# mizeller/OnePose_ST

Hardware: AMD Instinct MI355X
Metric: query frames/sec (2D-3D match+PnP) @ 7k x 4800 d256; 1/2/4/8 GPU (higher is better)
Workload: dtype bf16x3 (split-bf16 MFMA, f32 accumulate)

## Files before the change

onepose_st_amd/csrc/frame.hip:

```cpp
#include "tile.h"
#include "onepose_hip.h"
#include "x3w8_internal.h"
#include <mutex>
#include <unordered_map>
#include <vector>

namespace {

constexpr int kSlots = 16;
struct FineJob {
    bool pending = false;
    hipStream_t s_main = nullptr, s_fine = nullptr, s_copy = nullptr;
    const float* ff = nullptr; long long fs_b = 0, fs_c = 0, fs_y = 0, fs_x = 0; int hf = 0, wf = 0;
    const float* desc_f = nullptr; long long desc_f_bs = 0, desc_f_cs = 0;
    const long long *b_ids = nullptr, *i_ids = nullptr, *j_ids = nullptr; const int* count = nullptr; int cap = 0;
    const float* mkc = nullptr; const void* w_fine = nullptr; int n_fine = 0; unsigned fine_cross_bits = 0; int fine_encoder_enable = 0;
    int wc = 0, stride = 0; float fine_scale = 0.f;
    float *expec = nullptr, *mk2d = nullptr;
    const float* qscale = nullptr;
    void* host_dst = nullptr; const void* result_src = nullptr; size_t host_bytes = 0;
};
struct Slot {
    hipEvent_t prep_done = nullptr, coarse_done = nullptr, fine_done = nullptr, ready = nullptr, enc_done = nullptr;
    int dev = -1;
    int gen = 0;
    bool recorded = false;
    FineJob job;
};
struct DevState {
    Slot slots[kSlots];
    int next = 0;
    std::unordered_map<hipStream_t, hipEvent_t> last_fine;
    std::unordered_map<hipStream_t, int> deferred;
};
std::mutex g_mu;
std::mutex g_launch_mu;
std::unordered_map<int, DevState> g_dev;

size_t up256(size_t v) { return (v + 255) & ~(size_t)255; }

int make_events(Slot& s, int dev) {
    if (s.ready && s.dev == dev) return 0;
    hipEvent_t* ev[5] = {&s.prep_done, &s.coarse_done, &s.fine_done, &s.ready, &s.enc_done};
    for (auto e : ev) {
        hipError_t rc = hipEventCreateWithFlags(e, e == &s.ready ? (hipEventDisableTiming | hipEventBlockingSync) : hipEventDisableTiming);
        if (rc != hipSuccess) return ophip_fail(rc, "hipEventCreateWithFlags(frame)");
    }
    s.dev = dev;
    return 0;
}

}

#define FR_CHECK(call)                                  \
    do {                                                \
        const int rc__ = (call);                        \
        if (rc__ != 0) return rc__;                     \
    } while (0)
#define FR_HIP(call, what)                              \
    do {                                                \
        const hipError_t e__ = (call);                  \
        if (e__ != hipSuccess) return ophip_fail(e__, what); \
    } while (0)

namespace {
int launch_fine_job(int dev, Slot& s, hipEvent_t after = nullptr) {
    FineJob& j = s.job;
    const hipStream_t on = j.s_fine;
    FR_HIP(hipStreamWaitEvent(on, after ? after : s.coarse_done, 0), "hipStreamWaitEvent(fine job)");
    if (j.qscale)
        FR_CHECK(ophip_fine_refine_bf16_scaled(j.ff, j.fs_b, j.fs_c, j.fs_y, j.fs_x, j.hf, j.wf, j.desc_f, j.desc_f_bs, j.desc_f_cs, j.b_ids, j.i_ids, j.j_ids,
                                               j.count, j.cap, j.mkc, j.w_fine, j.n_fine, j.fine_cross_bits, j.fine_encoder_enable, 3, j.wc, j.stride,
                                               j.fine_scale, j.expec, j.mk2d, nullptr, nullptr, j.qscale, on));
    else
    FR_CHECK(ophip_fine_refine_bf16(j.ff, j.fs_b, j.fs_c, j.fs_y, j.fs_x, j.hf, j.wf, j.desc_f, j.desc_f_bs, j.desc_f_cs, j.b_ids, j.i_ids, j.j_ids,
                                    j.count, j.cap, j.mkc, j.w_fine, j.n_fine, j.fine_cross_bits, j.fine_encoder_enable, 3, j.wc, j.stride,
                                    j.fine_scale, j.expec, j.mk2d, nullptr, nullptr, on));
    FR_HIP(hipEventRecord(s.fine_done, on), "hipEventRecord(fine)");
    FR_HIP(hipStreamWaitEvent(j.s_copy, s.fine_done, 0), "hipStreamWaitEvent(fine)");
    FR_HIP(hipMemcpyAsync(j.host_dst, j.result_src, j.host_bytes, hipMemcpyDeviceToHost, j.s_copy), "hipMemcpyAsync(result block)");
// ... 72 lines not shown
    L->feat2d_out = (d->n_coarse % 2 == 0) ? L->x2d : L->y2d;
    return 0;
}

namespace {
int frame_enqueue_impl(const ophip_frame_desc* d, const ophip_frame_layout_t* L, void* blob_,
                       const float* feat_c, const float* feat_f, long long fs_b, long long fs_c, long long fs_y, long long fs_x,
                       const float* kpts, long long kpts_bs, const float* desc_c, long long desc_c_bs,
                       const float* desc_f, long long desc_f_bs, long long desc_f_cs, const ophip_object_cache* obj, bool ext_main_only,
                       const unsigned char* qmask, const float* qscale,
                       void* host_dst, size_t host_bytes, void* s_main_, void* s_prep_, void* s_fine_, void* s_copy_,
                       int* slot_out) {
    if (!d || !L || !blob_ || !feat_c || !feat_f || !kpts || !desc_c || !desc_f || !host_dst || !s_fine_ || !s_copy_ || !slot_out)
        return ophip_bad_arg(__func__, "null pointer");
    if (host_bytes < 16 || host_bytes > L->result_bytes) return ophip_bad_arg(__func__, "host_bytes");
    const bool deep = obj && obj->y3d0;
    const float* x3d_external = (obj && !deep) ? obj->x3d : nullptr;
    const long long x3d_ext_bs = obj ? obj->x3d_bs : -1;
    if (obj && !deep && !obj->x3d) return ophip_bad_arg(__func__, "object cache without buffers");
    if (deep && (!obj->kv1 || (reinterpret_cast<uintptr_t>(obj->kv1) & 15))) return ophip_bad_arg(__func__, "object cache: kv1 missing or not 16-byte aligned");
    if (deep && (d->n_coarse < 2 || (d->coarse_cross_bits & 1u))) return ophip_bad_arg(__func__, "a cached first layer needs n_coarse >= 2 and a first layer of kind \"self\"");
    if ((L->x3d == 0) != (obj != nullptr)) return ophip_bad_arg(__func__, "x3d_external / object cache does not match the layout");
    {
        const size_t want = deep ? ((d->n_coarse % 2 == 0) ? L->y3d : L->z3d) : ((d->n_coarse % 2 == 0) ? (obj ? L->z3d : L->x3d) : L->y3d);
        if (L->feat3d_out != want) return ophip_bad_arg(__func__, "layout was made for another external_x3d mode");
    }
    char* blob = static_cast<char*>(blob_);
    hipStream_t s_main = (hipStream_t)s_main_, s_prep = (hipStream_t)s_prep_, s_fine = (hipStream_t)s_fine_, s_copy = (hipStream_t)s_copy_;
    const int B = d->B, N = d->N, M = d->M, cap = B * N;
    int dev = 0;
    FR_HIP(hipGetDevice(&dev), "hipGetDevice");
    const bool defer = defer_fine_enabled() && s_fine != s_main;
    std::lock_guard<std::mutex> launch_lock(g_launch_mu);
    Slot* slot;
    Slot* kept = nullptr;
// ... 8 lines not shown
        slot = &st.slots[idx];
        FR_CHECK(make_events(*slot, dev));
        stale_job = slot->job.pending;
    }
    if (stale_job) FR_CHECK(launch_fine_job(dev, *slot));
    {
        std::lock_guard<std::mutex> lk(g_mu);
        DevState& st = g_dev[dev];
        if (slot->recorded) prev_ready = slot->ready;
        auto it = st.last_fine.find(s_main);
        if (it != st.last_fine.end()) prev_fine = it->second;
        auto dt = st.deferred.find(s_main);
        if (dt != st.deferred.end()) kept = &st.slots[dt->second];
    }
    if (prev_ready) FR_HIP(hipEventSynchronize(prev_ready), "hipEventSynchronize(slot reuse)");
    {
        std::lock_guard<std::mutex> lk(g_mu);
        slot->recorded = false;
        gen = ++slot->gen;
    }
    struct AbandonGuard {
        Slot* slot; hipStream_t st[4]; bool armed = true;
        ~AbandonGuard() {
            if (!armed) return;
            for (hipStream_t s : st) if (s) (void)hipStreamSynchronize(s);
            std::lock_guard<std::mutex> lk(g_mu);
            slot->recorded = false;
            slot->job.pending = false;
        }
    } abandon{slot, {s_main, s_prep, s_fine, s_copy}};
    auto F = [&](size_t off) { return reinterpret_cast<float*>(blob + off); };
    auto I64 = [&](size_t off) { return reinterpret_cast<long long*>(blob + off); };

    hipStream_t sin = s_prep ? s_prep : s_main;
    OphipRange frame_range("ophip_frame_enqueue");
    struct StageRange {
        bool open = false;
        void next(const char* name) { if (open) ophip_range_pop(); ophip_range_push(name); open = true; }
        ~StageRange() { if (open) ophip_range_pop(); }
    } stage;
    stage.next("a1-a3 input kernels");
    static const bool prep_after_sim = [] { const char* e = getenv("OPHIP_FRAME_PREP_AFTER_SIM"); return e && e[0] == '1'; }();
    if (prep_after_sim && s_prep && kept) FR_HIP(hipStreamWaitEvent(s_prep, kept->enc_done, 0), "hipStreamWaitEvent(previous similarity)");
    float* x2d = F(L->x2d);
    FR_CHECK(ophip_pe_add_transpose(feat_c, d->pe, x2d, B, 256, M, sin));
    const float* ff = feat_f;
    if (L->ffcl) {
        FR_CHECK(ophip_transpose_cl(feat_f, F(L->ffcl), B, d->cf, d->hf * d->wf, sin));
        ff = F(L->ffcl);
        fs_b = (long long)d->hf * d->wf * d->cf; fs_c = 1; fs_y = (long long)d->wf * d->cf; fs_x = d->cf;
    }
    if (obj && obj->ready) {
        FR_HIP(hipStreamWaitEvent(s_main, (hipEvent_t)obj->ready, 0), "hipStreamWaitEvent(object cache)");
        if (s_prep) FR_HIP(hipStreamWaitEvent(s_prep, (hipEvent_t)obj->ready, 0), "hipStreamWaitEvent(object cache, input stream)");
    }
    float* x3d = x3d_external ? const_cast<float*>(x3d_external) : (deep ? nullptr : F(L->x3d));
    if (!obj) {
        if (d->w_kpt) FR_CHECK(ophip_kpt_encode(kpts, kpts_bs, desc_c, desc_c_bs, d->w_kpt, F(L->stats), x3d, B, N, sin));
// ... 158 lines not shown
extern "C" int ophip_frame_enqueue(const ophip_frame_desc* d, const ophip_frame_layout_t* L, void* blob,
                                   const float* feat_c, const float* feat_f, long long fs_b, long long fs_c, long long fs_y, long long fs_x,
                                   const float* kpts, long long kpts_bs, const float* desc_c, long long desc_c_bs,
                                   const float* desc_f, long long desc_f_bs, long long desc_f_cs, const float* x3d_external,
                                   void* host_dst, size_t host_bytes, void* s_main, void* s_prep, void* s_fine, void* s_copy, int* slot_out) {
    return ophip_frame_enqueue_padded(d, L, blob, feat_c, feat_f, fs_b, fs_c, fs_y, fs_x, kpts, kpts_bs, desc_c, desc_c_bs, desc_f, desc_f_bs, desc_f_cs,
                                      x3d_external, nullptr, nullptr, host_dst, host_bytes, s_main, s_prep, s_fine, s_copy, slot_out);
}

extern "C" int ophip_frame_enqueue_object(const ophip_frame_desc* d, const ophip_frame_layout_t* L, void* blob,
                                          const float* feat_c, const float* feat_f, long long fs_b, long long fs_c, long long fs_y, long long fs_x,
                                          const float* kpts, long long kpts_bs, const float* desc_c, long long desc_c_bs,
                                          const float* desc_f, long long desc_f_bs, long long desc_f_cs, const ophip_object_cache* object,
                                          const unsigned char* qmask, const float* qscale,
                                          void* host_dst, size_t host_bytes, void* s_main, void* s_prep, void* s_fine, void* s_copy, int* slot_out) {
    if (object && !object->x3d && !object->y3d0) return ophip_bad_arg(__func__, "object cache without buffers");
    return frame_enqueue_impl(d, L, blob, feat_c, feat_f, fs_b, fs_c, fs_y, fs_x, kpts, kpts_bs, desc_c, desc_c_bs, desc_f, desc_f_bs, desc_f_cs,
                              object, false, qmask, qscale, host_dst, host_bytes, s_main, s_prep, s_fine, s_copy, slot_out);
}

extern "C" int ophip_frame_wait(int ticket) {
    if (ticket < kSlots) return ophip_bad_arg(__func__, "not a ticket of ophip_frame_enqueue");
    const int slot = ticket % kSlots, gen = ticket / kSlots;
    int dev = 0;
    FR_HIP(hipGetDevice(&dev), "hipGetDevice");
    hipEvent_t ev;
    {
        std::lock_guard<std::mutex> launch_lock(g_launch_mu);
        Slot* kept = nullptr;
        {
            std::lock_guard<std::mutex> lk(g_mu);
            Slot& s = g_dev[dev].slots[slot];
            if (s.gen > gen) return 0;
            if (s.gen == gen && s.job.pending) kept = &s;
        }
        if (kept) FR_CHECK(launch_fine_job(dev, *kept));
    }
    {
        std::lock_guard<std::mutex> lk(g_mu);
        const Slot& s = g_dev[dev].slots[slot];
        if (s.gen > gen) return 0;
        if (s.gen < gen || !s.recorded) return ophip_bad_arg(__func__, "ticket of a frame that was never (completely) enqueued on this device");
        ev = s.ready;
    }
    FR_HIP(hipEventSynchronize(ev), "hipEventSynchronize(frame)");
    return 0;
}

extern "C" int ophip_frame_order_after_fine(void* compute_stream) {
    int dev = 0;
    FR_HIP(hipGetDevice(&dev), "hipGetDevice");
    hipEvent_t ev = nullptr;
    std::lock_guard<std::mutex> launch_lock(g_launch_mu);
    Slot* kept = nullptr;
    {
        std::lock_guard<std::mutex> lk(g_mu);
        DevState& st = g_dev[dev];
        auto dt = st.deferred.find((hipStream_t)compute_stream);
        if (dt != st.deferred.end()) kept = &st.slots[dt->second];
    }
// ... 11 lines not shown
```

onepose_st_amd/csrc/prep.hip:

```cpp
#include "tile.h"
#include "crop_pixel.h"

namespace {

__global__ __launch_bounds__(256) void pe_add_transpose_kernel(const float* __restrict__ feat, const float* __restrict__ pe,
                                                               float* __restrict__ out, int Cc, int M) {
    __shared__ float tile[32][33];
    const int tx = threadIdx.x & 31, ty = threadIdx.x >> 5;
    const int m0 = blockIdx.x * 32, c0 = blockIdx.y * 32, b = blockIdx.z;
    const float* f = feat + (size_t)b * Cc * M;
#pragma unroll
    for (int k = 0; k < 4; ++k) {
        const int c = c0 + ty + 8 * k, m = m0 + tx;
        tile[ty + 8 * k][tx] = (c < Cc && m < M) ? f[(size_t)c * M + m] : 0.f;
    }
    __syncthreads();
    float* o = out + (size_t)b * M * Cc;
#pragma unroll
    for (int k = 0; k < 4; ++k) {
        const int m = m0 + ty + 8 * k, c = c0 + tx;
        if (m < M && c < Cc) o[(size_t)m * Cc + c] = tile[tx][ty + 8 * k] + (pe ? pe[(size_t)m * Cc + c] : 0.f);
    }
}

// ... 172 lines not shown
        for (int m = 0; m < 4; ++m) {
            const int q = q0 + 8 * m;
            f32x4 v = {tile[4 * q][p], tile[4 * q + 1][p], tile[4 * q + 2][p], tile[4 * q + 3][p]};
            *reinterpret_cast<f32x4*>(dst + (size_t)(l0 + p) * 128 + 4 * q) = v;
        }
    }
}

__global__ __launch_bounds__(256) void crop_resize_kernel(const unsigned char* __restrict__ img, int H, int W, int x0, int y0, int wb, int hb,
                                                          int S, float* __restrict__ out) {
    const int X = blockIdx.x * 32 + (threadIdx.x & 31), Y = blockIdx.y * 8 + (threadIdx.x >> 5);
    if (X >= S || Y >= S) return;
    out[(size_t)Y * S + X] = crop_pixel(img, H, W, x0, y0, wb, hb, S, X, Y);
}

}

extern "C" int ophip_crop_resize_gray(const unsigned char* image, int H, int W, int x0, int y0, int x1, int y1, int S, float* out, void* stream) {
    if (!image || !out) return ophip_bad_arg(__func__, "null pointer");
    if (H < 1 || W < 1 || S < 1 || x1 <= x0 || y1 <= y0) return ophip_bad_arg(__func__, "bad sizes (need x1 > x0, y1 > y0)");
    OPHIP_LAUNCH("crop_resize", (hipStream_t)stream, crop_resize_kernel, dim3((S + 31) / 32, (S + 7) / 8), dim3(256), 0, (hipStream_t)stream,
                 image, H, W, x0, y0, x1 - x0, y1 - y0, S, out);
    OPHIP_CHECK_LAUNCH();
    return 0;
}

extern "C" int ophip_pe_add_transpose(const float* feat_nchw, const float* pe_nlc, float* out_nlc, int B, int C, int M, void* stream) {
    if (!feat_nchw || !out_nlc) return ophip_bad_arg(__func__, "null pointer");
    if (B < 1 || C < 1 || M < 1) return ophip_bad_arg(__func__, "bad sizes");
    OPHIP_LAUNCH("pe_add_transpose", (hipStream_t)stream, pe_add_transpose_kernel, dim3((M + 31) / 32, (C + 31) / 32, B), dim3(256), 0, (hipStream_t)stream,
// ... 40 lines not shown
```

onepose_st_amd/csrc/x3w8_internal.h:

```cpp
#pragma once

int ophip_x3w8_object_first(const float* x2d, float* y2d, int B, int L3d, int L2d, const void* wpack, const void* wpack_next, int kv_mode,
                            void* workspace, const unsigned char* mask2d, bool only_kv, void* stream);
int ophip_x3w8_object_second(const float* y3d0, long long y3d0_bs, const float* x2d, float* y3d, float* y2d, int B, int L3d, int L2d,
                             const void* wpack, const void* wpack_next, int is_cross, const void* kv1, long long kv1_bs,
                             void* workspace, void* frag3d, void* frag2d, const unsigned char* mask2d, void* stream);
int ophip_x3w8_layer_bs(const float* x3d, long long x3d_bs, const float* x2d, float* y3d, float* y2d, int B, int L3d, int L2d,
                        const void* wpack, const void* wpack_next, int is_cross, int kv_mode, int slot,
                        void* workspace, void* frag3d, void* frag2d, const unsigned char* mask2d, bool only_kv, void* stream);

bool ophip_coarse_two_pass(int B, int N, int M);

int ophip_coarse_sim_store(const float* feat0, const float* feat1, int B, int N, int M, float* conf, float* workspace,
                           const float** rowstat, float** rowbest, unsigned** colmax_bits, void* stream,
                           const unsigned char* mask0 = nullptr, const unsigned char* mask1 = nullptr);
int ophip_coarse_select_2d(const float* conf, int nspan, const float* points0, long long points_bstride, int B, int N, int M, int wi, int wc,
                           float thr, int border_rm, float scale, float* workspace, long long* b_ids, long long* i_ids, long long* j_ids,
                           float* mconf, float* mkpts0, float* mkpts1_c, long long* m_bids, unsigned char* gt_mask, int* count, void* stream,
                           const unsigned char* mask0 = nullptr, const unsigned char* mask1 = nullptr);
```

onepose_st_amd/model.py:

```python
from __future__ import annotations

import contextlib
import ctypes
import os
import weakref
from collections import namedtuple

import torch
import torch.nn as nn

from . import hip, host_math, ops, packing
from .backbone import build_backbone
from .backbone_hip import HipBackbone, pack_backbone
from .config import encoder_layer_names, validate_config
from .hip import bstride
from .lazy_conf import LazyConfMatrixBase
from .params import EncoderParams, load_matcher_checkpoint
from .rows import rows_encoder_layer


class _KeypointEncoderParams(nn.Module):

    def __init__(self, inp_dim, feature_dim, layers):
        super().__init__()
# ... 11 lines not shown


def _current_stream(dev):
    idx = dev.index
    if idx is None:
        return torch.cuda.current_stream(dev)
    raw = torch._C._cuda_getCurrentRawStream(idx)
    st = _stream_objs.get((idx, raw))
    if st is None:
        st = torch.cuda.current_stream(dev)
        if len(_stream_objs) >= 64:
            _stream_objs.clear()
        _stream_objs[(idx, raw)] = st
    return st


_NSPLIT = {"f32": 0, "bf16": 1, "bf16x3": 3}


def _side_stream(table, key, dev, priority=0, with_event=False):
    ent = table.get(key)
    if ent is None:
        if len(table) >= 16:
            table.pop(next(iter(table)))
        st = torch.cuda.Stream(device=dev, priority=priority)
        ent = table[key] = [st, None] if with_event else st
    return ent


def _dense(t):
# ... 54 lines not shown
        fp = config.get("hip_fine_precision")
        if fp is not None:
            if str(fp) not in ("bf16x3", "bf16"):
                raise ValueError(f"hip_fine_precision {fp!r}: expected 'bf16x3' or 'bf16'")
            os.environ["OPHIP_FINE_PRECISION"] = str(fp)
        self.hip_backbone = bool(config.get("hip_backbone", True)) and self.precision != "f32"
        self.lazy_reruns = 0
        self._packed = None
        self._packed_bb = None
        self.overlap_fine = bool(config.get("hip_overlap_fine", True))
        self._fine_streams = {}
        self._prep_streams = {}
        self._pe_cache = {}
        self.cache_object = bool(config.get("hip_cache_object", False))
        self._obj_cache = None
        self.conf_matrix_mode = str(config.get("hip_conf_matrix", "eager"))
        if self.conf_matrix_mode not in ("eager", "lazy"):
            raise ValueError(f"hip_conf_matrix {self.conf_matrix_mode!r}: expected 'eager' or 'lazy'")
        if self.conf_matrix_mode == "lazy" and self.precision == "f32":
            raise ValueError("hip_conf_matrix = 'lazy' needs a bf16 arithmetic mode (the exact-f32 mode always materialises conf_matrix)")
        self.frame_call = bool(config.get("hip_frame_call", os.environ.get("OPHIP_FRAME_CALL", "1") != "0"))
        self._frame_plans = {}
        self._plan_ids = set()
        weakref.finalize(self, ops.drop_frame_plans, self._plan_ids)
        self._frame_call_pending = set()

        pretrained = config["loftr_backbone"]["pretrained"]
        if pretrained is not None:
            ckpt = torch.load(pretrained, map_location="cpu", weights_only=True)["state_dict"]
            sub = {k[k.find("backbone") + len("backbone") + 1:]: v for k, v in ckpt.items() if "backbone" in k}
# ... 55 lines not shown

        def coarse(pack):
            return [pack(sd, f"loftr_coarse.layers.{i}.").to(device) for i in range(len(self.loftr_coarse.layer_names))]
        blocks = {"coarse": coarse(packing.pack_coarse_layer),
                  "fine": torch.cat([packing.pack_fine_layer(sd, f"loftr_fine.layers.{i}.") for i in range(n_fine)]).to(device)}
        if self.kpt_3d_pos_encoding is not None:
            blocks["kpt"] = packing.pack_keypoint_encoder(sd).to(device)
        if self.precision == "bf16":
            blocks["coarse_bf16"] = coarse(packing.pack_coarse_layer_bf16)
        if self.precision == "bf16x3":
            blocks["coarse_x3"] = coarse(packing.pack_coarse_layer_x3w8)
        if self.fine_full:
            blocks["fine_full"] = [{n: t.to(device) for n, t in packing.pack_fine_layer_full_x3(sd, f"loftr_fine.layers.{i}.").items()} for i in range(n_fine)]
        if self.precision != "f32":
            blocks["fine_bf16"] = packing.pack_fine_layers_bf16(sd, "loftr_fine.layers.", n_fine).to(device)
        self._packed = (key, blocks)
        return blocks

    def _backbone_blocks(self, device):
        tensors = list(self.backbone.state_dict().values())
        key = (str(device),) + tuple((t.data_ptr(), t._version) for t in tensors)
        if self._packed_bb is None or self._packed_bb[0] != key:
            self._packed_bb = (key, pack_backbone(self.backbone.state_dict(), device))
        return self._packed_bb[1]

    def _pe_table(self, h, w, device):
        k = (h, w, str(device))
        if k not in self._pe_cache:
            self._pe_cache[k] = host_math.pe_table(self.config["loftr_coarse"]["d_model"], h, w, self._pe_shape).to(device)
        return self._pe_cache[k]
# ... 20 lines not shown
        if not self.hip_backbone:
            raise RuntimeError("hip_backbone is disabled for this model (exact-f32 mode or config['hip_backbone'] = False)")
        if not img.is_cuda:
            raise hip.HipLibraryError("OnePosePlus_model runs on the HIP device only (no CPU fallback): move the "
                                      "model and its inputs to 'cuda'")
        B, _, H, W = img.shape
        pe = self._pe_table(H // 8, W // 8, img.device) if self._pe_enable else None
        fc, ff = HipBackbone(self.precision).forward(self._backbone_blocks(img.device), img, pe)
        return (fc.view(B, H // 8, W // 8, fc.shape[2]).permute(0, 3, 1, 2), ff.view(B, H // 2, W // 2, ff.shape[2]).permute(0, 3, 1, 2))

    def forward_features(self, data, feat_c, feat_f, image_hw=None, want_fine_debug=False):
        self.enqueue_features(data, feat_c, feat_f, image_hw, want_fine_debug).finish()

    @torch.no_grad()
    def enqueue_features(self, data, feat_c, feat_f, image_hw=None, want_fine_debug=False, host_copy=False, _pe_applied=False,
                         inputs_ready=False, _force_eager=False):
        fi = self._frame_inputs(data, feat_c, feat_f, image_hw)
        main = _current_stream(fi.dev)
        fkey = (str(fi.dev), main.cuda_stream)
        lazy = self.conf_matrix_mode == "lazy" and not _force_eager
        rerun = (lambda: self.enqueue_features(data, feat_c, feat_f, image_hw, want_fine_debug, host_copy, _pe_applied, False, True)) if lazy else None
        if (self.frame_call and self.precision == "bf16x3" and not self.coarse_full and not self.fine_full and self.overlap_fine and not _pe_applied and not want_fine_debug
                and not self.debug and bool(self.config["fine_matching"]["enable"])
                and (self.kpt_3d_pos_encoding is not None or fi.B == 1 or fi.desc_in_d.shape[0] == fi.B)
                and len(self.loftr_coarse.layer_names) <= 16):
            return self._enqueue_frame_call(data, feat_c, feat_f, fi, main, fkey, host_copy, inputs_ready, lazy, rerun)
        if fkey in self._frame_call_pending:
            self._frame_call_pending.discard(fkey)
            hip.call("ophip_frame_order_after_fine", ctypes.c_void_p(main.cuda_stream))
        x2d, x3d, ff, ff_strides = self._input_stage(fi, feat_c, feat_f, main, fkey, _pe_applied, inputs_ready)
        x3d, x2d = self._coarse_encoder_stage(fi, x3d, x2d, main, fkey)
        if self.debug:
            data["_feat3d_c"], data["_feat2d_c"] = x3d, x2d
        cb, select = self._coarse_matching_stage(data, fi, x3d, x2d, main, lazy)
        pend = self._fine_stage(data, fi, cb, select, ff, ff_strides, main, fkey, want_fine_debug, host_copy)
        pend._rerun = rerun
        return pend

    def _frame_inputs(self, data, feat_c, feat_f, image_hw):
        if not feat_c.is_cuda:
            raise hip.HipLibraryError("OnePosePlus_model runs on the HIP device only (no CPU fallback): move the "
# ... 301 lines not shown
            d.w_kpt = W["kpt"].data_ptr() if self.kpt_3d_pos_encoding is not None else None
            for li in range(len(names_c)):
                d.w_coarse[li] = W["coarse_x3"][li].data_ptr()
            d.w_fine = W["fine_bf16"].data_ptr()
            L = hip.FrameLayout()
            hip.call("ophip_frame_layout", ctypes.byref(d), 1 if transpose_fine else 0, ext_mode, ctypes.byref(L))
            if len(self._frame_plans) >= 8:
                old_id = self._frame_plans.pop(next(iter(self._frame_plans)))[2]
                self._plan_ids.discard(old_id)
                ops.drop_frame_plan(old_id)
            pid = ops.register_frame_plan(d, L, keep_alive=(W, pe))
            self._plan_ids.add(pid)
            plan = self._frame_plans[pkey] = (d, L, pid, (W, pe))
        return plan

    def _enqueue_frame_call(self, data, feat_c, feat_f, fi, main, fkey, host_copy, inputs_ready, lazy=False, rerun=None):
        B, N, M, dev, kpts_d, desc_in_d, desc_fine_d, qmask, qscale = fi.B, fi.N, fi.M, fi.dev, fi.kpts_d, fi.desc_in_d, fi.desc_fine_d, fi.qmask, fi.qscale
        x3d_ext = None
        if self.cache_object or (B > 1 and kpts_d.shape[0] == 1 and desc_in_d.shape[0] == 1):
            x3d_ext = self._object_cache_entry(fi, main, masked=qmask is not None, keep=self.cache_object)
        fc = _dense(feat_c)
        ff = feat_f if feat_f.dtype == torch.float32 else feat_f.float()
        transpose_fine = ff.stride(1) != 1
        if transpose_fine:
            ff = ff.contiguous()
        ext_mode = 0 if x3d_ext is None else (2 if x3d_ext["y3d0"] is not None else 1)
        d, L, plan_id = self._frame_plan(fi, ff.shape[1], transpose_fine, ext_mode, data["q_hw_i"][0], lazy)[:3]

        fine_entry = self._fine_streams.get(fkey)
        if fine_entry is None:
            fine_entry = _side_stream(self._fine_streams, fkey, dev, int(os.environ.get("OPHIP_FINE_PRIO", "0")), with_event=True)
        elif fine_entry[1] is not None:
            main.wait_event(fine_entry[1])
            fine_entry[1] = None
        sfine = fine_entry[0]
        sprep = _side_stream(self._prep_streams, fkey, dev) if inputs_ready else None
        scopy = _side_stream(PendingFrame._copy_streams, (dev, main.cuda_stream), dev)
        cap = B * N
        if sprep is not None:
            with torch.cuda.stream(sprep):
                blob = torch.empty(L.total, dtype=torch.uint8, device=dev)
        else:
            blob = torch.empty(L.total, dtype=torch.uint8, device=dev)
        for st in (sfine, scopy) if sprep is None else (main, sfine, scopy):
            blob.record_stream(st)
        nbytes = int(L.result_bytes) if host_copy else 16
        pin = PendingFrame._take_pin((cap, bool(host_copy)), nbytes)
        fs = (0, 0, 0, 0) if transpose_fine else (ff.stride(0), 1, ff.stride(2), ff.stride(3))
        try:
            with self.profiler.record_function("LoFTR/coarse-matching/get_coarse_match"), \
                    self.profiler.record_function("LoFTR/coarse-matching/get_coarse_match/argmax-conf"):
                oc = x3d_ext or {"x3d": None, "y3d0": None, "kv1": None, "ev": None}
                slot = torch.ops.onepose_hip.frame_enqueue(plan_id, blob, fc, ff, list(fs), kpts_d, desc_in_d, desc_fine_d, oc["x3d"], pin, nbytes,
                                                           main.cuda_stream, sprep.cuda_stream if sprep is not None else 0,
                                                           sfine.cuda_stream, scopy.cuda_stream, qmask, qscale, oc["y3d0"], oc["kv1"],
                                                           oc["ev"].cuda_event if oc["ev"] is not None else 0)
        except Exception:
            torch.cuda.synchronize(dev)
            PendingFrame._pinned_pool.setdefault((cap, bool(host_copy)), []).append(pin)
            raise
        self._frame_call_pending.add(fkey)
        if lazy:
            f3 = blob[L.feat3d_out:L.feat3d_out + 4 * B * N * 256].view(torch.float32).view(B, N, 256)
            f2 = blob[L.feat2d_out:L.feat2d_out + 4 * B * M * 256].view(torch.float32).view(B, M, 256)
            data["conf_matrix"] = LazyConfMatrix(f3, f2, float(self.config["coarse_matching"]["dual_softmax"]["temperature"]), _NSPLIT["bf16x3"], main, qmask)
        else:
            data["conf_matrix"] = blob[L.conf:L.conf + 4 * B * N * M].view(torch.float32).view(B, N, M)
        keep = [fc, ff, kpts_d, desc_in_d, desc_fine_d, x3d_ext, fi.W, qmask, qscale]
        pend = PendingFrame._from_block(self, data, dev, B, N, M, cap, blob, L, slot, pin, host_copy, keep)
        pend._rerun = rerun
        return pend


class LazyConfMatrix(LazyConfMatrixBase):

    def __init__(self, feat3d, feat2d, temperature, nsplit, stream, query_mask=None):
        super().__init__((feat3d.shape[0], feat3d.shape[1], feat2d.shape[1]), feat3d.device)
        self._f3, self._f2, self._temp, self._nsplit, self._stream, self._qmask = feat3d, feat2d, temperature, nsplit, stream, query_mask

    def _compute(self) -> torch.Tensor:
        B, N, M = self.shape
        dev = self.device
        cur = torch.cuda.current_stream(dev)
        cur.wait_stream(self._stream)
        conf = torch.empty(B, N, M, device=dev, dtype=torch.float32)
# ... 24 lines not shown

    _pinned_pool = {}
    _copy_streams = {}

    def __init__(self, model, data, dev, B, N, M, cap, fine_on, want_dbg, bufs, host_copy):
        self.model, self.data, self.dev = model, data, dev
        self.B, self.N, self.M, self.cap, self.fine_on, self.want_dbg = B, N, M, cap, fine_on, want_dbg
        self.bufs = bufs
        self.host = None
        key = (cap, bool(host_copy))
        nbytes = bufs["blob"].numel() if host_copy else 16
        self._pin = PendingFrame._take_pin(key, nbytes)
        self._key, self._host_copy = key, bool(host_copy)
        self._slot = None
        self._rerun = None
        main = torch.cuda.current_stream(dev)
        side = _side_stream(PendingFrame._copy_streams, (dev, main.cuda_stream), dev)
        ready = torch.cuda.Event()
        ready.record(main)
        side.wait_event(ready)
        self.event = torch.cuda.Event()
        with torch.cuda.stream(side):
            self._pin.copy_(bufs["blob"][:nbytes], non_blocking=True)
            self.event.record(side)
        self.done = False

    @staticmethod
    def _take_pin(key, nbytes):
        pool = PendingFrame._pinned_pool.setdefault(key, [])
        return pool.pop() if pool else torch.empty(nbytes, dtype=torch.uint8).pin_memory()

    @classmethod
    def _from_block(cls, model, data, dev, B, N, M, cap, blob, layout, slot, pin, host_copy, keep):
        self = cls.__new__(cls)
        self.model, self.data, self.dev = model, data, dev
        self.B, self.N, self.M, self.cap, self.fine_on, self.want_dbg = B, N, M, cap, True, False
        self.bufs, self.host = None, None
        self._block, self._layout, self._slot, self._keep = blob, layout, slot, keep
        self._pin, self._key, self._host_copy = pin, (cap, bool(host_copy)), bool(host_copy)
        self.event = None
        self._rerun = None
        self.done = False
        return self

    def wait(self):
        self._wait()

    def _wait(self):
        if self._slot is not None:
            hip.call("ophip_frame_wait", self._slot)
        else:
            self.event.synchronize()

    def _block_views(self):
        blob, L, cap = self._block, self._layout, self.cap
        res = blob[L.result:L.result + L.result_bytes]
# ... 21 lines not shown
        finally:
            self._release_pin()
            self.done = True

    def __del__(self):
        try:
            self.close()
        except Exception:
            pass

    def finish(self, on_host=None):
        if self.done:
            return self.data
        self._wait()
        K = int(self._pin[:4].view(torch.int32)[0])
        if self._rerun is not None and int(self._pin[4:8].view(torch.int32)[0]) != 0:
            self._release_pin()
            self.done = True
            self.model.lazy_reruns += 1
            again = self._rerun()
            again.finish(on_host)
            self.host = again.host
            return self.data
        B, N, M, cap = self.B, self.N, self.M, self.cap
        if self._host_copy:
            _, _, hb, h3, h2 = _result_views(self._pin, cap)
            self.host = {"K": K, "mkpts_3d_db": h3[:K].numpy().copy(), "mkpts_2d": h2[:K].numpy().copy(), "b_ids": hb[:K].numpy().copy()}
            if on_host is not None:
                on_host(self.host)
        self._release_pin()
# ... 30 lines not shown
```

onepose_st_amd/ops.py:

```python
from __future__ import annotations

import ctypes
import itertools

import torch

from . import hip

_lib = torch.library.Library("onepose_hip", "DEF")

_lib.define("pe_add_transpose(Tensor feat_nchw, Tensor? pe_nlc, Tensor(a!) out_nlc) -> ()")
_lib.define("kpt_encode(Tensor keypoints3d, Tensor desc_bcn, Tensor wpack, Tensor(a!) out_bnc) -> ()")
_lib.define("encoder_layer_x3w8(Tensor x3d, Tensor x2d, Tensor(a!) y3d, Tensor(b!) y2d, Tensor wpack, Tensor? wpack_next, "
            "bool is_cross, bool kv_from_prev, int slot, Tensor(c!) workspace) -> ()")
_lib.define("encoder_layer_x3w8_frag(Tensor x3d, Tensor x2d, Tensor(a!) y3d, Tensor(b!) y2d, Tensor wpack, Tensor? wpack_next, "
            "bool is_cross, bool kv_from_prev, int slot, Tensor(c!) workspace, Tensor(d!) coarse_workspace) -> ()")
_lib.define("coarse_match(Tensor feat3d, Tensor feat2d, Tensor keypoints3d, int wc, float temperature, float thr, int border_rm, "
            "float scale, int nsplit) -> (Tensor, Tensor, Tensor, Tensor, Tensor, Tensor, Tensor, Tensor)")
_lib.define("fine_refine_bf16(Tensor feat_f_cl, Tensor desc3d_f, Tensor b_ids, Tensor i_ids, Tensor j_ids, Tensor count, Tensor mkpts_c, "
            "Tensor wpack, int nlayers, int cross_bits, bool encoder_enable, int nsplit, int wc, int stride, float fine_scale) -> (Tensor, Tensor)")
_lib.define("frame_enqueue(int plan, Tensor(a!) block, Tensor feat_c, Tensor feat_f, int[] fine_strides, Tensor keypoints3d, "
            "Tensor desc3d_c, Tensor desc3d_f, Tensor? x3d_external, Tensor(b!) host_dst, int host_bytes, "
            "int s_main, int s_prep, int s_fine, int s_copy, Tensor? query_mask=None, Tensor? query_scale=None, "
            "Tensor? y3d0=None, Tensor? kv1=None, int object_ready=0) -> int")


def _f32(t: torch.Tensor, name: str) -> torch.Tensor:
    if not t.is_cuda or t.dtype != torch.float32 or not t.is_contiguous():
        raise ValueError(f"{name}: expected a contiguous float32 tensor on the HIP device")
    return t


def _pe_add_transpose(feat_nchw, pe_nlc, out_nlc):
    B, C, h, w = feat_nchw.shape
    hip.call("ophip_pe_add_transpose", hip.ptr(_f32(feat_nchw, "feat_nchw")), hip.ptr(pe_nlc), hip.ptr(_f32(out_nlc, "out_nlc")), B, C, h * w,
             hip.stream_handle())


def _kpt_encode(keypoints3d, desc_bcn, wpack, out_bnc):
# ... 71 lines not shown
    pid = next(_plan_ids)
    _frame_plans[pid] = (desc, layout, keep_alive)
    return pid


def drop_frame_plan(pid: int):
    _frame_plans.pop(pid, None)


def drop_frame_plans(pids):
    for pid in list(pids):
        _frame_plans.pop(pid, None)


def _frame_enqueue(plan, block, feat_c, feat_f, fine_strides, keypoints3d, desc3d_c, desc3d_f, x3d_external, host_dst, host_bytes,
                   s_main, s_prep, s_fine, s_copy, query_mask=None, query_scale=None, y3d0=None, kv1=None, object_ready=0):
    if plan not in _frame_plans:
        raise ValueError(f"frame plan {plan} is not registered (ops.register_frame_plan)")
    d, L = _frame_plans[plan][:2]
    if block.numel() * block.element_size() < L.total:
        raise ValueError(f"block: {L.total} bytes needed (ophip_frame_layout)")
    if host_dst.is_cuda or not host_dst.is_pinned():
        raise ValueError("host_dst must be pinned host memory")
    fs = list(fine_strides)
    if len(fs) != 4:
        raise ValueError("fine_strides: 4 element strides (b, c, y, x)")
    slot = ctypes.c_int(-1)
    vp = ctypes.c_void_p
    CALLS["frame_enqueue"] += 1
    if query_mask is not None and (query_mask.dtype != torch.uint8 or tuple(query_mask.shape) != (d.B, d.M) or not query_mask.is_contiguous()):
        raise ValueError("query_mask: contiguous uint8 [B, M]")
# ... 6 lines not shown
        oc = hip.ObjectCache()
        for t, name in ((x3d_external, "x3d_external"), (y3d0, "y3d0")):
            if t is not None and (t.dtype != torch.float32 or not t.is_cuda or not t.is_contiguous() or t.dim() != 3
                                  or t.shape[0] not in (1, d.B) or tuple(t.shape[1:]) != (d.N, 256)):
                raise ValueError(f"{name}: contiguous float32 [1 or B, N, 256] on the HIP device")
        if x3d_external is not None:
            oc.x3d, oc.x3d_bs = x3d_external.data_ptr(), (0 if (x3d_external.shape[0] == 1 and d.B > 1) else d.N * 256)
        if y3d0 is not None:
            kvb = hip.load().ophip_encoder_x3w8_kv_block_bytes()
            if kv1.dtype != torch.uint8 or not kv1.is_cuda or not kv1.is_contiguous() or tuple(kv1.shape) != (y3d0.shape[0], kvb):
                raise ValueError(f"kv1: contiguous uint8 [{y3d0.shape[0]}, {kvb}] on the HIP device")
            shared = y3d0.shape[0] == 1 and d.B > 1
            oc.y3d0, oc.y3d0_bs = y3d0.data_ptr(), (0 if shared else d.N * 256)
            oc.kv1, oc.kv1_bs = kv1.data_ptr(), (0 if shared else kvb)
        oc.ready = int(object_ready) or None
    hip.call("ophip_frame_enqueue_object", ctypes.byref(d), ctypes.byref(L), vp(block.data_ptr()),
             hip.ptr(feat_c), hip.ptr(feat_f), fs[0], fs[1], fs[2], fs[3], hip.ptr(keypoints3d), hip.bstride(keypoints3d),
             hip.ptr(desc3d_c), hip.bstride(desc3d_c), hip.ptr(desc3d_f), hip.bstride(desc3d_f), desc3d_f.stride(1), ctypes.byref(oc) if oc is not None else None,
             hip.ptr(query_mask, torch.uint8), hip.ptr(query_scale), vp(host_dst.data_ptr()), int(host_bytes), vp(s_main), vp(s_prep) if s_prep else None, vp(s_fine), vp(s_copy), ctypes.byref(slot))
    return slot.value


_lib.impl("pe_add_transpose", _pe_add_transpose, "CUDA")
_lib.impl("kpt_encode", _kpt_encode, "CUDA")
_lib.impl("encoder_layer_x3w8", _encoder_layer_x3w8, "CUDA")
_lib.impl("encoder_layer_x3w8_frag", _encoder_layer_x3w8_frag, "CUDA")
_lib.impl("coarse_match", _coarse_match, "CUDA")
_lib.impl("fine_refine_bf16", _fine_refine_bf16, "CUDA")
_lib.impl("frame_enqueue", _frame_enqueue, "CUDA")

# ... 2 lines not shown
```

Measured before the change: 1503.

## Cache object-side encoder outputs across frames with on-device verification and rerun

```diff
diff --git a/onepose_st_amd/csrc/frame.hip b/onepose_st_amd/csrc/frame.hip
--- a/onepose_st_amd/csrc/frame.hip
+++ b/onepose_st_amd/csrc/frame.hip
@@ -25,6 +25,8 @@
     int dev = -1;
     int gen = 0;
     bool recorded = false;
+    unsigned long long obj_serial = 0;
+    const unsigned* host_word = nullptr;
     FineJob job;
 };
 struct DevState {
@@ -39,6 +41,41 @@
 
 size_t up256(size_t v) { return (v + 255) & ~(size_t)255; }
 
+constexpr int kObjEntries = 4;
+constexpr int kObjModeX3 = 3;
+struct ObjKey {
+    const float* kpts = nullptr; long long kpts_bs = 0; const float* desc = nullptr; long long desc_bs = 0;
+    int N = 0, masked = 0, mode = 0;
+    const void *w_kpt = nullptr, *w0 = nullptr, *w1 = nullptr; long long pack_version = 0;
+    bool operator==(const ObjKey& o) const {
+        return kpts == o.kpts && kpts_bs == o.kpts_bs && desc == o.desc && desc_bs == o.desc_bs && N == o.N && masked == o.masked && mode == o.mode &&
+               w_kpt == o.w_kpt && w0 == o.w0 && w1 == o.w1 && pack_version == o.pack_version;
+    }
+};
+struct ObjEntry {
+    bool valid = false;
+    unsigned long long serial = 0, last_used = 0;
+    ObjKey key;
+    char* mem = nullptr; size_t mem_bytes = 0;
+    size_t o_sdesc = 0, o_skpts = 0, o_x3d = 0, o_y3d0 = 0, o_kv1 = 0, o_stats = 0, o_ws = 0;
+    hipEvent_t ready = nullptr; bool ready_seen = false;
+};
+struct ObjTable { ObjEntry e[kObjEntries]; unsigned long long clock = 0; };
+std::mutex g_obj_mu;
+std::unordered_map<int, ObjTable> g_obj;
+unsigned long long g_obj_serial = 0;
+
+void object_drop(int dev, unsigned long long serial) {
+    std::lock_guard<std::mutex> lk(g_obj_mu);
+    for (ObjEntry& e : g_obj[dev].e)
+        if (e.serial == serial) e.valid = false;
+}
+void object_check_slot(int dev, Slot& s) {
+    if (s.obj_serial && s.host_word && *s.host_word) object_drop(dev, s.obj_serial);
+    s.obj_serial = 0;
+    s.host_word = nullptr;
+}
+
 int make_events(Slot& s, int dev) {
     if (s.ready && s.dev == dev) return 0;
     hipEvent_t* ev[5] = {&s.prep_done, &s.coarse_done, &s.fine_done, &s.ready, &s.enc_done};
@@ -64,6 +101,68 @@
     } while (0)
 
 namespace {
+int object_find_or_build(int dev, const ObjKey& key, const ophip_frame_desc* d, hipStream_t s_main, ophip_object_cache* oc, bool* hit,
+                         unsigned long long* serial, const float** snap_kpts, const float** snap_desc) {
+    ObjEntry* ent = nullptr;
+    {
+        std::lock_guard<std::mutex> lk(g_obj_mu);
+        ObjTable& t = g_obj[dev];
+        for (ObjEntry& e : t.e)
+            if (e.valid && e.key == key) ent = &e;
+        *hit = ent != nullptr;
+        if (!ent) {
+            for (ObjEntry& e : t.e)
+                if (!ent || (!e.valid && ent->valid) || (e.valid == ent->valid && e.last_used < ent->last_used)) ent = &e;
+            ent->valid = false;
+        }
+        ent->last_used = ++t.clock;
+    }
+    const size_t N = key.N, rows = N * 256 * sizeof(float);
+    if (!*hit) {
+        ObjEntry& e = *ent;
+        size_t o = 0;
+        auto take = [&](size_t bytes) { const size_t at = o; o = up256(o + bytes); return at; };
+        e.o_sdesc = take(rows); e.o_skpts = take(N * 3 * sizeof(float)); e.o_x3d = take(rows); e.o_y3d0 = take(rows);
+        e.o_kv1 = take(ophip_encoder_x3w8_kv_block_bytes()); e.o_stats = take(8 * sizeof(float));
+        e.o_ws = take(ophip_encoder_x3w8_workspace_bytes(1, key.N, 1));
+        if (e.mem) FR_HIP(hipDeviceSynchronize(), "hipDeviceSynchronize(object entry reuse)");
+        if (e.mem_bytes < o) {
+            if (e.mem) FR_HIP(hipFree(e.mem), "hipFree(object entry)");
+            e.mem = nullptr; e.mem_bytes = 0;
+            FR_HIP(hipMalloc(reinterpret_cast<void**>(&e.mem), o), "hipMalloc(object entry)");
+            e.mem_bytes = o;
+        }
+        if (!e.ready) FR_HIP(hipEventCreateWithFlags(&e.ready, hipEventDisableTiming), "hipEventCreateWithFlags(object entry)");
+        float *sdesc = reinterpret_cast<float*>(e.mem + e.o_sdesc), *skpts = reinterpret_cast<float*>(e.mem + e.o_skpts);
+        float *x3d = reinterpret_cast<float*>(e.mem + e.o_x3d), *y3d0 = reinterpret_cast<float*>(e.mem + e.o_y3d0);
+        OphipRange range("object entry build");
+        FR_HIP(hipMemcpyAsync(sdesc, key.desc, rows, hipMemcpyDeviceToDevice, s_main), "hipMemcpyAsync(object snapshot)");
+        FR_HIP(hipMemcpyAsync(skpts, key.kpts, N * 3 * sizeof(float), hipMemcpyDeviceToDevice, s_main), "hipMemcpyAsync(object snapshot)");
+        if (d->w_kpt) FR_CHECK(ophip_kpt_encode(skpts, 0, sdesc, 0, d->w_kpt, reinterpret_cast<float*>(e.mem + e.o_stats), x3d, 1, key.N, s_main));
+        else FR_CHECK(ophip_transpose_cl(sdesc, x3d, 1, 256, key.N, s_main));
+        FR_CHECK(ophip_encoder_object_x3w8(x3d, 1, key.N, d->w_coarse[0], d->w_coarse[1], e.mem + e.o_ws, y3d0, e.mem + e.o_kv1, key.masked, s_main));
+        FR_HIP(hipEventRecord(e.ready, s_main), "hipEventRecord(object entry)");
+        std::lock_guard<std::mutex> lk(g_obj_mu);
+        e.key = key;
+        e.serial = ++g_obj_serial;
+        e.ready_seen = false;
+        e.valid = true;
+    }
+    ObjEntry& e = *ent;
+    if (!e.ready_seen) {
+        if (hipEventQuery(e.ready) == hipSuccess) e.ready_seen = true;
+        else (void)hipGetLastError();
+    }
+    oc->x3d = reinterpret_cast<const float*>(e.mem + e.o_x3d); oc->x3d_bs = (long long)N * 256;
+    oc->y3d0 = reinterpret_cast<const float*>(e.mem + e.o_y3d0); oc->y3d0_bs = (long long)N * 256;
+    oc->kv1 = e.mem + e.o_kv1; oc->kv1_bs = (long long)ophip_encoder_x3w8_kv_block_bytes();
+    oc->ready = e.ready_seen ? nullptr : e.ready;
+    *serial = e.serial;
+    *snap_kpts = reinterpret_cast<const float*>(e.mem + e.o_skpts);
+    *snap_desc = reinterpret_cast<const float*>(e.mem + e.o_sdesc);
+    return 0;
+}
+
 int launch_fine_job(int dev, Slot& s, hipEvent_t after = nullptr) {
     FineJob& j = s.job;
     const hipStream_t on = j.s_fine;
@@ -166,11 +265,15 @@
     if (!d || !L || !blob_ || !feat_c || !feat_f || !kpts || !desc_c || !desc_f || !host_dst || !s_fine_ || !s_copy_ || !slot_out)
         return ophip_bad_arg(__func__, "null pointer");
     if (host_bytes < 16 || host_bytes > L->result_bytes) return ophip_bad_arg(__func__, "host_bytes");
-    const bool deep = obj && obj->y3d0;
+    const bool automatic = obj && !obj->x3d && !obj->y3d0 && !obj->kv1;
+    const long long pack_version = automatic ? obj->x3d_bs : 0;
+    if (automatic && (d->B != 1 || obj->ready || kpts_bs != 0 || desc_c_bs != 0))
+        return ophip_bad_arg(__func__, "the object table serves one frame per call with an object block of its own (B = 1, batch strides 0, no event)");
+    const bool deep = automatic || (obj && obj->y3d0);
     const float* x3d_external = (obj && !deep) ? obj->x3d : nullptr;
-    const long long x3d_ext_bs = obj ? obj->x3d_bs : -1;
+    const long long x3d_ext_bs = (obj && !automatic) ? obj->x3d_bs : -1;
     if (obj && !deep && !obj->x3d) return ophip_bad_arg(__func__, "object cache without buffers");
-    if (deep && (!obj->kv1 || (reinterpret_cast<uintptr_t>(obj->kv1) & 15))) return ophip_bad_arg(__func__, "object cache: kv1 missing or not 16-byte aligned");
+    if (deep && !automatic && (!obj->kv1 || (reinterpret_cast<uintptr_t>(obj->kv1) & 15))) return ophip_bad_arg(__func__, "object cache: kv1 missing or not 16-byte aligned");
     if (deep && (d->n_coarse < 2 || (d->coarse_cross_bits & 1u))) return ophip_bad_arg(__func__, "a cached first layer needs n_coarse >= 2 and a first layer of kind \"self\"");
     if ((L->x3d == 0) != (obj != nullptr)) return ophip_bad_arg(__func__, "x3d_external / object cache does not match the layout");
     {
@@ -209,6 +312,7 @@
         if (dt != st.deferred.end()) kept = &st.slots[dt->second];
     }
     if (prev_ready) FR_HIP(hipEventSynchronize(prev_ready), "hipEventSynchronize(slot reuse)");
+    { std::lock_guard<std::mutex> lk(g_mu); object_check_slot(dev, *slot); }
     {
         std::lock_guard<std::mutex> lk(g_mu);
         slot->recorded = false;
@@ -222,6 +326,8 @@
             std::lock_guard<std::mutex> lk(g_mu);
             slot->recorded = false;
             slot->job.pending = false;
+            slot->obj_serial = 0;
+            slot->host_word = nullptr;
         }
     } abandon{slot, {s_main, s_prep, s_fine, s_copy}};
     auto F = [&](size_t off) { return reinterpret_cast<float*>(blob + off); };
@@ -237,6 +343,23 @@
     stage.next("a1-a3 input kernels");
     static const bool prep_after_sim = [] { const char* e = getenv("OPHIP_FRAME_PREP_AFTER_SIM"); return e && e[0] == '1'; }();
     if (prep_after_sim && s_prep && kept) FR_HIP(hipStreamWaitEvent(s_prep, kept->enc_done, 0), "hipStreamWaitEvent(previous similarity)");
+    ophip_object_cache oc_auto{};
+    if (automatic) {
+        unsigned* word = reinterpret_cast<unsigned*>(blob + L->result) + 2;
+        FR_CHECK(ophip_frame_head(word, sin));
+        ObjKey key;
+        key.kpts = kpts; key.kpts_bs = kpts_bs; key.desc = desc_c; key.desc_bs = desc_c_bs; key.N = N; key.masked = qmask ? 1 : 0; key.mode = kObjModeX3;
+        key.w_kpt = d->w_kpt; key.w0 = d->w_coarse[0]; key.w1 = d->w_coarse[1]; key.pack_version = pack_version;
+        bool hit = false;
+        unsigned long long serial = 0;
+        const float *snap_kpts = nullptr, *snap_desc = nullptr;
+        FR_CHECK(object_find_or_build(dev, key, d, s_main, &oc_auto, &hit, &serial, &snap_kpts, &snap_desc));
+        if (hit && oc_auto.ready) FR_HIP(hipStreamWaitEvent(sin, (hipEvent_t)oc_auto.ready, 0), "hipStreamWaitEvent(object entry)");
+        if (hit) FR_CHECK(ophip_object_verify(desc_c, snap_desc, (long long)N * 256, kpts, snap_kpts, (long long)N * 3, word, sin));
+        obj = &oc_auto;
+        slot->obj_serial = serial;
+        slot->host_word = reinterpret_cast<const unsigned*>(static_cast<const char*>(host_dst)) + 2;
+    }
     float* x2d = F(L->x2d);
     FR_CHECK(ophip_pe_add_transpose(feat_c, d->pe, x2d, B, 256, M, sin));
     const float* ff = feat_f;
@@ -425,7 +548,7 @@
                                           const float* desc_f, long long desc_f_bs, long long desc_f_cs, const ophip_object_cache* object,
                                           const unsigned char* qmask, const float* qscale,
                                           void* host_dst, size_t host_bytes, void* s_main, void* s_prep, void* s_fine, void* s_copy, int* slot_out) {
-    if (object && !object->x3d && !object->y3d0) return ophip_bad_arg(__func__, "object cache without buffers");
+    if (object && !object->x3d && !object->y3d0 && object->kv1) return ophip_bad_arg(__func__, "object cache without buffers");
     return frame_enqueue_impl(d, L, blob, feat_c, feat_f, fs_b, fs_c, fs_y, fs_x, kpts, kpts_bs, desc_c, desc_c_bs, desc_f, desc_f_bs, desc_f_cs,
                               object, false, qmask, qscale, host_dst, host_bytes, s_main, s_prep, s_fine, s_copy, slot_out);
 }
@@ -455,6 +578,11 @@
         ev = s.ready;
     }
     FR_HIP(hipEventSynchronize(ev), "hipEventSynchronize(frame)");
+    {
+        std::lock_guard<std::mutex> lk(g_mu);
+        Slot& s = g_dev[dev].slots[slot];
+        if (s.gen == gen) object_check_slot(dev, s);
+    }
     return 0;
 }
 
diff --git a/onepose_st_amd/csrc/prep.hip b/onepose_st_amd/csrc/prep.hip
--- a/onepose_st_amd/csrc/prep.hip
+++ b/onepose_st_amd/csrc/prep.hip
@@ -1,5 +1,6 @@
 #include "tile.h"
 #include "crop_pixel.h"
+#include "x3w8_internal.h"
 
 namespace {
 
@@ -210,6 +211,56 @@
     out[(size_t)Y * S + X] = crop_pixel(img, H, W, x0, y0, wb, hb, S, X, Y);
 }
 
+__global__ void frame_head_kernel(unsigned* __restrict__ word) {
+    if (threadIdx.x == 0) *word = 0u;
+}
+
+constexpr int OV_THREADS = 256, OV_F4_PER_THREAD = 4, OV_MAX_BLOCKS = 1024;
+
+__device__ __forceinline__ unsigned verify_segment(const float* __restrict__ live, const float* __restrict__ snap, unsigned n, bool vec, unsigned t, unsigned T) {
+    unsigned d = 0u;
+    const unsigned n4 = vec ? n / 4 : 0;
+    const uint4* __restrict__ l4 = reinterpret_cast<const uint4*>(live);
+    const uint4* __restrict__ s4 = reinterpret_cast<const uint4*>(snap);
+#pragma unroll 2
+    for (unsigned i = t; i < n4; i += T) {
+        const uint4 a = l4[i], b = s4[i];
+        d |= (a.x ^ b.x) | (a.y ^ b.y) | (a.z ^ b.z) | (a.w ^ b.w);
+    }
+    for (unsigned k = 4 * n4 + t; k < n; k += T) d |= __float_as_uint(live[k]) ^ __float_as_uint(snap[k]);
+    return d;
+}
+
+__global__ __launch_bounds__(OV_THREADS) void object_verify_kernel(const float* __restrict__ desc_live, const float* __restrict__ desc_snap, long long n_desc, int desc_vec,
+                                                                   const float* __restrict__ kpts_live, const float* __restrict__ kpts_snap, long long n_kpts, int kpts_vec,
+                                                                   unsigned* __restrict__ word) {
+    const unsigned t = blockIdx.x * OV_THREADS + threadIdx.x, T = gridDim.x * OV_THREADS;
+    const unsigned d = verify_segment(desc_live, desc_snap, (unsigned)n_desc, desc_vec != 0, t, T) |
+                       verify_segment(kpts_live, kpts_snap, (unsigned)n_kpts, kpts_vec != 0, t, T);
+    if (d) *word = *word | 1u;
+}
+
+}
+
+int ophip_frame_head(unsigned* word, void* stream) {
+    if (!word) return ophip_bad_arg(__func__, "null pointer");
+    OPHIP_LAUNCH("frame_head", (hipStream_t)stream, frame_head_kernel, dim3(1), dim3(64), 0, (hipStream_t)stream, word);
+    OPHIP_CHECK_LAUNCH();
+    return 0;
+}
+
+int ophip_object_verify(const float* desc_live, const float* desc_snap, long long n_desc, const float* kpts_live, const float* kpts_snap,
+                        long long n_kpts, unsigned* word, void* stream) {
+    if (!desc_live || !desc_snap || !kpts_live || !kpts_snap || !word) return ophip_bad_arg(__func__, "null pointer");
+    if (n_desc < 0 || n_kpts < 0 || n_desc >= (1ll << 31) || n_kpts >= (1ll << 31)) return ophip_bad_arg(__func__, "bad sizes");
+    auto aligned = [](const float* a, const float* b) { return ((reinterpret_cast<uintptr_t>(a) | reinterpret_cast<uintptr_t>(b)) & 15) == 0; };
+    const long long per_block = (long long)OV_THREADS * OV_F4_PER_THREAD * 4;
+    long long blocks = (n_desc + n_kpts + per_block - 1) / per_block;
+    blocks = blocks < 1 ? 1 : (blocks > OV_MAX_BLOCKS ? OV_MAX_BLOCKS : blocks);
+    OPHIP_LAUNCH("object_verify", (hipStream_t)stream, object_verify_kernel, dim3((unsigned)blocks), dim3(OV_THREADS), 0, (hipStream_t)stream,
+                 desc_live, desc_snap, n_desc, aligned(desc_live, desc_snap) ? 1 : 0, kpts_live, kpts_snap, n_kpts, aligned(kpts_live, kpts_snap) ? 1 : 0, word);
+    OPHIP_CHECK_LAUNCH();
+    return 0;
 }
 
 extern "C" int ophip_crop_resize_gray(const unsigned char* image, int H, int W, int x0, int y0, int x1, int y1, int S, float* out, void* stream) {
diff --git a/onepose_st_amd/csrc/x3w8_internal.h b/onepose_st_amd/csrc/x3w8_internal.h
--- a/onepose_st_amd/csrc/x3w8_internal.h
+++ b/onepose_st_amd/csrc/x3w8_internal.h
@@ -9,6 +9,10 @@
                         const void* wpack, const void* wpack_next, int is_cross, int kv_mode, int slot,
                         void* workspace, void* frag3d, void* frag2d, const unsigned char* mask2d, bool only_kv, void* stream);
 
+int ophip_frame_head(unsigned* word, void* stream);
+int ophip_object_verify(const float* desc_live, const float* desc_snap, long long n_desc, const float* kpts_live, const float* kpts_snap,
+                        long long n_kpts, unsigned* word, void* stream);
+
 bool ophip_coarse_two_pass(int B, int N, int M);
 
 int ophip_coarse_sim_store(const float* feat0, const float* feat1, int B, int N, int M, float* conf, float* workspace,
diff --git a/onepose_st_amd/model.py b/onepose_st_amd/model.py
--- a/onepose_st_amd/model.py
+++ b/onepose_st_amd/model.py
@@ -2,6 +2,7 @@
 
 import contextlib
 import ctypes
+import itertools
 import os
 import weakref
 from collections import namedtuple
@@ -49,6 +50,8 @@
         _stream_objs[(idx, raw)] = st
     return st
 
+
+_pack_versions = itertools.count(1)
 
 _NSPLIT = {"f32": 0, "bf16": 1, "bf16x3": 3}
 
@@ -133,6 +136,10 @@
         self._pe_cache = {}
         self.cache_object = bool(config.get("hip_cache_object", False))
         self._obj_cache = None
+        self.object_reuse = str(config.get("hip_object_reuse", "auto"))
+        if self.object_reuse not in ("auto", "off"):
+            raise ValueError(f"hip_object_reuse {self.object_reuse!r}: expected 'auto' or 'off'")
+        self.object_reruns = 0
         self.conf_matrix_mode = str(config.get("hip_conf_matrix", "eager"))
         if self.conf_matrix_mode not in ("eager", "lazy"):
             raise ValueError(f"hip_conf_matrix {self.conf_matrix_mode!r}: expected 'eager' or 'lazy'")
@@ -218,6 +225,7 @@
             blocks["fine_full"] = [{n: t.to(device) for n, t in packing.pack_fine_layer_full_x3(sd, f"loftr_fine.layers.{i}.").items()} for i in range(n_fine)]
         if self.precision != "f32":
             blocks["fine_bf16"] = packing.pack_fine_layers_bf16(sd, "loftr_fine.layers.", n_fine).to(device)
+        blocks["pack_version"] = next(_pack_versions)
         self._packed = (key, blocks)
         return blocks
 
@@ -268,17 +276,21 @@
 
     @torch.no_grad()
     def enqueue_features(self, data, feat_c, feat_f, image_hw=None, want_fine_debug=False, host_copy=False, _pe_applied=False,
-                         inputs_ready=False, _force_eager=False):
+                         inputs_ready=False, _force_eager=False, _object_reuse=True):
         fi = self._frame_inputs(data, feat_c, feat_f, image_hw)
         main = _current_stream(fi.dev)
         fkey = (str(fi.dev), main.cuda_stream)
         lazy = self.conf_matrix_mode == "lazy" and not _force_eager
-        rerun = (lambda: self.enqueue_features(data, feat_c, feat_f, image_hw, want_fine_debug, host_copy, _pe_applied, False, True)) if lazy else None
+        rerun = (lambda: self.enqueue_features(data, feat_c, feat_f, image_hw, want_fine_debug, host_copy, _pe_applied, False, True, _object_reuse)) if lazy else None
         if (self.frame_call and self.precision == "bf16x3" and not self.coarse_full and not self.fine_full and self.overlap_fine and not _pe_applied and not want_fine_debug
                 and not self.debug and bool(self.config["fine_matching"]["enable"])
                 and (self.kpt_3d_pos_encoding is not None or fi.B == 1 or fi.desc_in_d.shape[0] == fi.B)
                 and len(self.loftr_coarse.layer_names) <= 16):
-            return self._enqueue_frame_call(data, feat_c, feat_f, fi, main, fkey, host_copy, inputs_ready, lazy, rerun)
+            pend = self._enqueue_frame_call(data, feat_c, feat_f, fi, main, fkey, host_copy, inputs_ready, lazy, rerun, _object_reuse)
+            if pend._object_word:
+                pend._rerun_object = lambda: self.enqueue_features(data, feat_c, feat_f, image_hw, want_fine_debug, host_copy, _pe_applied, False,
+                                                                   _force_eager, False)
+            return pend
         if fkey in self._frame_call_pending:
             self._frame_call_pending.discard(fkey)
             hip.call("ophip_frame_order_after_fine", ctypes.c_void_p(main.cuda_stream))
@@ -610,17 +622,20 @@
             plan = self._frame_plans[pkey] = (d, L, pid, (W, pe))
         return plan
 
-    def _enqueue_frame_call(self, data, feat_c, feat_f, fi, main, fkey, host_copy, inputs_ready, lazy=False, rerun=None):
+    def _enqueue_frame_call(self, data, feat_c, feat_f, fi, main, fkey, host_copy, inputs_ready, lazy=False, rerun=None, object_reuse=True):
         B, N, M, dev, kpts_d, desc_in_d, desc_fine_d, qmask, qscale = fi.B, fi.N, fi.M, fi.dev, fi.kpts_d, fi.desc_in_d, fi.desc_fine_d, fi.qmask, fi.qscale
         x3d_ext = None
         if self.cache_object or (B > 1 and kpts_d.shape[0] == 1 and desc_in_d.shape[0] == 1):
             x3d_ext = self._object_cache_entry(fi, main, masked=qmask is not None, keep=self.cache_object)
+        names = self.loftr_coarse.layer_names
+        auto = (object_reuse and x3d_ext is None and self.object_reuse == "auto" and B == 1 and len(names) >= 2 and names[0] == "self"
+                and kpts_d is data["keypoints3d"] and desc_in_d is data.get("descriptors3d_coarse_db", data["descriptors3d_db"]))
         fc = _dense(feat_c)
         ff = feat_f if feat_f.dtype == torch.float32 else feat_f.float()
         transpose_fine = ff.stride(1) != 1
         if transpose_fine:
             ff = ff.contiguous()
-        ext_mode = 0 if x3d_ext is None else (2 if x3d_ext["y3d0"] is not None else 1)
+        ext_mode = (2 if auto else 0) if x3d_ext is None else (2 if x3d_ext["y3d0"] is not None else 1)
         d, L, plan_id = self._frame_plan(fi, ff.shape[1], transpose_fine, ext_mode, data["q_hw_i"][0], lazy)[:3]
 
         fine_entry = self._fine_streams.get(fkey)
@@ -650,7 +665,8 @@
                 slot = torch.ops.onepose_hip.frame_enqueue(plan_id, blob, fc, ff, list(fs), kpts_d, desc_in_d, desc_fine_d, oc["x3d"], pin, nbytes,
                                                            main.cuda_stream, sprep.cuda_stream if sprep is not None else 0,
                                                            sfine.cuda_stream, scopy.cuda_stream, qmask, qscale, oc["y3d0"], oc["kv1"],
-                                                           oc["ev"].cuda_event if oc["ev"] is not None else 0)
+                                                           oc["ev"].cuda_event if oc["ev"] is not None else 0,
+                                                           fi.W["pack_version"] if auto else 0)
         except Exception:
             torch.cuda.synchronize(dev)
             PendingFrame._pinned_pool.setdefault((cap, bool(host_copy)), []).append(pin)
@@ -665,6 +681,7 @@
         keep = [fc, ff, kpts_d, desc_in_d, desc_fine_d, x3d_ext, fi.W, qmask, qscale]
         pend = PendingFrame._from_block(self, data, dev, B, N, M, cap, blob, L, slot, pin, host_copy, keep)
         pend._rerun = rerun
+        pend._object_word = auto
         return pend
 
 
@@ -719,6 +736,7 @@
         self._key, self._host_copy = key, bool(host_copy)
         self._slot = None
         self._rerun = None
+        self._rerun_object, self._object_word = None, False
         main = torch.cuda.current_stream(dev)
         side = _side_stream(PendingFrame._copy_streams, (dev, main.cuda_stream), dev)
         ready = torch.cuda.Event()
@@ -745,6 +763,7 @@
         self._pin, self._key, self._host_copy = pin, (cap, bool(host_copy)), bool(host_copy)
         self.event = None
         self._rerun = None
+        self._rerun_object, self._object_word = None, False
         self.done = False
         return self
 
@@ -796,6 +815,14 @@
             return self.data
         self._wait()
         K = int(self._pin[:4].view(torch.int32)[0])
+        if self._object_word and int(self._pin[8:12].view(torch.int32)[0]) != 0:
+            self._release_pin()
+            self.done = True
+            self.model.object_reruns += 1
+            again = self._rerun_object()
+            again.finish(on_host)
+            self.host = again.host
+            return self.data
         if self._rerun is not None and int(self._pin[4:8].view(torch.int32)[0]) != 0:
             self._release_pin()
             self.done = True
diff --git a/onepose_st_amd/ops.py b/onepose_st_amd/ops.py
--- a/onepose_st_amd/ops.py
+++ b/onepose_st_amd/ops.py
@@ -22,7 +22,7 @@
 _lib.define("frame_enqueue(int plan, Tensor(a!) block, Tensor feat_c, Tensor feat_f, int[] fine_strides, Tensor keypoints3d, "
             "Tensor desc3d_c, Tensor desc3d_f, Tensor? x3d_external, Tensor(b!) host_dst, int host_bytes, "
             "int s_main, int s_prep, int s_fine, int s_copy, Tensor? query_mask=None, Tensor? query_scale=None, "
-            "Tensor? y3d0=None, Tensor? kv1=None, int object_ready=0) -> int")
+            "Tensor? y3d0=None, Tensor? kv1=None, int object_ready=0, int object_pack_version=0) -> int")
 
 
 def _f32(t: torch.Tensor, name: str) -> torch.Tensor:
@@ -124,7 +124,7 @@
 
 
 def _frame_enqueue(plan, block, feat_c, feat_f, fine_strides, keypoints3d, desc3d_c, desc3d_f, x3d_external, host_dst, host_bytes,
-                   s_main, s_prep, s_fine, s_copy, query_mask=None, query_scale=None, y3d0=None, kv1=None, object_ready=0):
+                   s_main, s_prep, s_fine, s_copy, query_mask=None, query_scale=None, y3d0=None, kv1=None, object_ready=0, object_pack_version=0):
     if plan not in _frame_plans:
         raise ValueError(f"frame plan {plan} is not registered (ops.register_frame_plan)")
     d, L = _frame_plans[plan][:2]
@@ -161,6 +161,9 @@
             oc.y3d0, oc.y3d0_bs = y3d0.data_ptr(), (0 if shared else d.N * 256)
             oc.kv1, oc.kv1_bs = kv1.data_ptr(), (0 if shared else kvb)
         oc.ready = int(object_ready) or None
+    elif object_pack_version:
+        oc = hip.ObjectCache()
+        oc.x3d_bs = int(object_pack_version)
     hip.call("ophip_frame_enqueue_object", ctypes.byref(d), ctypes.byref(L), vp(block.data_ptr()),
              hip.ptr(feat_c), hip.ptr(feat_f), fs[0], fs[1], fs[2], fs[3], hip.ptr(keypoints3d), hip.bstride(keypoints3d),
              hip.ptr(desc3d_c), hip.bstride(desc3d_c), hip.ptr(desc3d_f), hip.bstride(desc3d_f), desc3d_f.stride(1), ctypes.byref(oc) if oc is not None else None,
```

Result: faster. 1541 (median of 6 runs) (+2.5%).
